# skitzoid/Box2D-MT

Hardware: AMD Instinct MI355X
Metric: world steps/sec at 99858 bodies per GPU (BASELINE config 3: Tumbler 100k, CCD off; Step = collide + island solve + broad-phase + state read-back); for N > 1: container-steps/s = world steps/s x N containers in the one sharded world (higher is better)
Workload: dtype f32

## Files before the change

### box2d-mt_amd/csrc/b2d_kernels_solve_large.h

```cpp
#ifndef B2D_KERNELS_SOLVE_LARGE_H
#define B2D_KERNELS_SOLVE_LARGE_H

#include "b2d_kernels_solve_small.h"

#define LC_WORDS ((int)(sizeof(ContactConstraint) / 4))
#define LC_VEL_WORDS 36
#define LC_IMP_FIRST 10
#define LC_MASS_FIRST 28
#define LC_POS_FIRST 36

__device__ __forceinline__ void lcStore(const DW& W, int row, const ContactConstraint& cc, int first, int last)
{
	uint32_t words[LC_WORDS];
	memcpy(words, &cc, sizeof(ContactConstraint));
	uint32_t* dst = (uint32_t*)W.lc;
#pragma unroll
	for (int f = 0; f < LC_WORDS; ++f)
	{
		if (f >= first && f < last) dst[(size_t)f * W.capContacts + row] = words[f];
	}
}

__device__ __forceinline__ void lcLoad(const DW& W, int row, ContactConstraint& cc, int first, int last)
{
// ... 345 lines not shown
	for (int s = blockIdx.x * blockDim.x + threadIdx.x; s < n; s += gridDim.x * blockDim.x)
	{
		if (W.li_color[s] >= 0) continue;
		const int ci = W.li_contacts[s];
		int4 ids = C.ids[ci];
		uint32_t pr = colorPriority(ci);
		if ((W.b_flags[ids.z] & BF_TYPE_MASK) != BT_STATIC) atomicMax(&W.bodyClaim[ids.z], pr);
		if ((W.b_flags[ids.w] & BF_TYPE_MASK) != BT_STATIC) atomicMax(&W.bodyClaim[ids.w], pr);
	}
}

__global__ __launch_bounds__(256) void k_color_resolve(DW W)
{
	b2dPhaseStamp(W);
	DState* S = W.st;
	if (S->c.nUncolored == 0) return;
	const int n = S->c.nLContacts;
	const ContactArrays& C = W.ca[S->cur];
	int colored = 0;
	for (int s = blockIdx.x * blockDim.x + threadIdx.x; s < n; s += gridDim.x * blockDim.x)
	{
		if (W.li_color[s] >= 0) continue;
		const int ci = W.li_contacts[s];
		int4 ids = C.ids[ci];
		uint32_t pr = colorPriority(ci);
		const bool nsA = (W.b_flags[ids.z] & BF_TYPE_MASK) != BT_STATIC;
		const bool nsB = (W.b_flags[ids.w] & BF_TYPE_MASK) != BT_STATIC;
		bool win = true;
		if (nsA && __hip_atomic_load(&W.bodyClaim[ids.z], __ATOMIC_RELAXED, __HIP_MEMORY_SCOPE_AGENT) != pr) win = false;
		if (nsB && __hip_atomic_load(&W.bodyClaim[ids.w], __ATOMIC_RELAXED, __HIP_MEMORY_SCOPE_AGENT) != pr) win = false;
		if (!win) continue;
		uint64_t used = colorClassMask(constraintIsCut(W, ids.z, nsA, ids.w, nsB)) | colorTestMask(W);
		if (nsA) used |= W.bodyColorMask[ids.z];
		if (nsB) used |= W.bodyColorMask[ids.w];
		int color = used == ~0ull ? MAX_COLORS - 1 : __ffsll((long long)~used) - 1;
		if (used == ~0ull) atomicOr(&S->c.overflow, 4);
		uint64_t bit = 1ull << color;
		if (nsA) { W.bodyColorMask[ids.z] |= bit; W.bodyClaim[ids.z] = 0; }
		if (nsB) { W.bodyColorMask[ids.w] |= bit; W.bodyClaim[ids.w] = 0; }
		W.li_color[s] = color;
		C.color[ci] = color;
		atomicAdd(&W.colorCount[colorSlot(color)], 1);
		atomicMax(&S->c.nColors, color + 1);
		noteColorUsed(S, color);
		++colored;
	}
	if (colored) atomicSub(&S->c.nUncolored, colored);
}

__host__ __device__ inline bool b2dColorAheadNoPartition(const Counters& c, int aheadMinRows)
{
	return aheadMinRows > 0 && c.nBlocks == 0 && c.nLContacts >= aheadMinRows;
}
__device__ __forceinline__ void colorSmallBody(const DW& W);
__global__ __launch_bounds__(1024) void k_color_small(DW W, int queuedAhead, int aheadMinRows, DState* pub, int pubSeq)
{
	b2dPhaseStamp(W);
	DState* S = W.st;
	if (threadIdx.x == 0) S->gapClock[2] = wall_clock64();
	bool run = true, publish = pub != nullptr;
	if (queuedAhead)
	{
		const bool noPart = b2dColorAheadNoPartition(S->c, aheadMinRows);
		run = b2dPartitionSettled(S->c) || noPart;
		publish = publish && noPart;
	}
	if (S->c.nUncolList > COLOR_SMALL_MAX || S->c.needRecolor) run = false;
	if (run) colorSmallBody(W);
	if (publish)
	{
		__syncthreads();
		if (run && threadIdx.x < MAX_COLORS) S->c.colorRows[threadIdx.x] = threadIdx.x == HUB_COLOR ? 0 : __hip_atomic_load(&W.colorCount[colorSlot(threadIdx.x)], __ATOMIC_RELAXED, __HIP_MEMORY_SCOPE_WORKGROUP);
		__syncthreads();
		b2dPublishCensus(W, pub, pubSeq);
	}
}
__device__ __forceinline__ void colorSmallBody(const DW& W)
{
	DState* S = W.st;
	const ContactArrays& C = W.ca[S->cur];
	__shared__ int s_left, s_colored, s_maxColor, s_n;
	if (threadIdx.x == 0)
	{
		s_n = S->c.nUncolList;
		s_maxColor = 0;
	}
	__syncthreads();
	{
		const int nc = S->c.nCompact + S->c.nUncolList <= COLOR_SMALL_MAX ? S->c.nCompact : 0;
		for (int k = threadIdx.x; k < nc; k += blockDim.x)
		{
			const int s = W.compactList[k];
			const int c = W.li_color[s];
			if (c <= 0 || c >= MAX_COLORS) continue;
			const int ci = W.li_contacts[s];
			const int4 ids = C.ids[ci];
			const bool nsA = (W.b_flags[ids.z] & BF_TYPE_MASK) != BT_STATIC;
			const bool nsB = (W.b_flags[ids.w] & BF_TYPE_MASK) != BT_STATIC;
			uint64_t used = colorClassMask(constraintIsCut(W, ids.z, nsA, ids.w, nsB)) | colorTestMask(W);
			if (nsA) used |= __hip_atomic_load((unsigned long long*)&W.bodyColorMask[ids.z], __ATOMIC_RELAXED, __HIP_MEMORY_SCOPE_WORKGROUP);
			if (nsB) used |= __hip_atomic_load((unsigned long long*)&W.bodyColorMask[ids.w], __ATOMIC_RELAXED, __HIP_MEMORY_SCOPE_WORKGROUP);
			if (used == ~0ull || __ffsll((long long)~used) - 1 >= c) continue;
			const int slot = atomicAdd(&s_n, 1);
			if (slot >= COLOR_SMALL_MAX) continue;
			const unsigned long long bit = 1ull << c;
			if (nsA) (void)__hip_atomic_fetch_and((unsigned long long*)&W.bodyColorMask[ids.z], ~bit, __ATOMIC_RELAXED, __HIP_MEMORY_SCOPE_WORKGROUP);
			if (nsB) (void)__hip_atomic_fetch_and((unsigned long long*)&W.bodyColorMask[ids.w], ~bit, __ATOMIC_RELAXED, __HIP_MEMORY_SCOPE_WORKGROUP);
			W.li_color[s] = -1;
			C.color[ci] = -1;
			(void)__hip_atomic_fetch_add(&W.colorCount[colorSlot(c)], -1, __ATOMIC_RELAXED, __HIP_MEMORY_SCOPE_WORKGROUP);
			W.uncolList[slot] = s;
		}
	}
	__syncthreads();
	const int n = s_n < COLOR_SMALL_MAX ? s_n : COLOR_SMALL_MAX;
	if (threadIdx.x == 0)
	{
		s_left = n;
		if (s_n > S->c.nUncolList) S->c.compactMoved = s_n - S->c.nUncolList;
	}
	constexpr int PER = COLOR_SMALL_MAX / 1024;
	int it_s[PER], it_ci[PER], it_a[PER], it_b[PER];
	uint32_t it_pr[PER];
	uint64_t it_class[PER];
	bool it_open[PER];
#pragma unroll
	for (int j = 0; j < PER; ++j)
	{
		const int k = (int)threadIdx.x + j * 1024;
		it_open[j] = false;
		it_s[j] = it_ci[j] = 0; it_a[j] = it_b[j] = -1; it_pr[j] = 0u; it_class[j] = 0ull;
		if (k < n)
		{
			const int s = W.uncolList[k];
			it_s[j] = s;
			it_open[j] = W.li_color[s] < 0;
			const int ci = W.li_contacts[s];
			it_ci[j] = ci;
			const int4 ids = C.ids[ci];
			const bool nsA = (W.b_flags[ids.z] & BF_TYPE_MASK) != BT_STATIC;
			const bool nsB = (W.b_flags[ids.w] & BF_TYPE_MASK) != BT_STATIC;
			it_a[j] = nsA ? ids.z : -1;
			it_b[j] = nsB ? ids.w : -1;
			it_pr[j] = colorPriority(ci);
			it_class[j] = colorClassMask(constraintIsCut(W, ids.z, nsA, ids.w, nsB)) | colorTestMask(W);
		}
	}
	__syncthreads();
	const int maxRounds = W.testColorRounds > 0 ? W.testColorRounds : 4 * MAX_COLORS;
	for (int round = 0; round < maxRounds && s_left > 0; ++round)
	{
		if (threadIdx.x == 0) s_colored = 0;
#pragma unroll
		for (int j = 0; j < PER; ++j)
		{
			if (!it_open[j]) continue;
			if (it_a[j] >= 0) (void)__hip_atomic_fetch_max(&W.bodyClaim[it_a[j]], it_pr[j], __ATOMIC_RELAXED, __HIP_MEMORY_SCOPE_WORKGROUP);
			if (it_b[j] >= 0) (void)__hip_atomic_fetch_max(&W.bodyClaim[it_b[j]], it_pr[j], __ATOMIC_RELAXED, __HIP_MEMORY_SCOPE_WORKGROUP);
		}
		__syncthreads();
		int colored = 0;
#pragma unroll
		for (int j = 0; j < PER; ++j)
		{
			if (!it_open[j]) continue;
			const int A = it_a[j], B = it_b[j];
			const uint32_t pr = it_pr[j];
			bool win = true;
			if (A >= 0 && __hip_atomic_load(&W.bodyClaim[A], __ATOMIC_RELAXED, __HIP_MEMORY_SCOPE_WORKGROUP) != pr) win = false;
			if (B >= 0 && __hip_atomic_load(&W.bodyClaim[B], __ATOMIC_RELAXED, __HIP_MEMORY_SCOPE_WORKGROUP) != pr) win = false;
			if (!win) continue;
			uint64_t used = it_class[j];
			if (A >= 0) used |= __hip_atomic_load((unsigned long long*)&W.bodyColorMask[A], __ATOMIC_RELAXED, __HIP_MEMORY_SCOPE_WORKGROUP);
			if (B >= 0) used |= __hip_atomic_load((unsigned long long*)&W.bodyColorMask[B], __ATOMIC_RELAXED, __HIP_MEMORY_SCOPE_WORKGROUP);
			const int color = used == ~0ull ? MAX_COLORS - 1 : __ffsll((long long)~used) - 1;
			if (used == ~0ull) atomicOr(&S->c.overflow, 4);
			const unsigned long long bit = 1ull << color;
			if (A >= 0) { (void)__hip_atomic_fetch_or((unsigned long long*)&W.bodyColorMask[A], bit, __ATOMIC_RELAXED, __HIP_MEMORY_SCOPE_WORKGROUP); __hip_atomic_store(&W.bodyClaim[A], 0u, __ATOMIC_RELAXED, __HIP_MEMORY_SCOPE_WORKGROUP); }
			if (B >= 0) { (void)__hip_atomic_fetch_or((unsigned long long*)&W.bodyColorMask[B], bit, __ATOMIC_RELAXED, __HIP_MEMORY_SCOPE_WORKGROUP); __hip_atomic_store(&W.bodyClaim[B], 0u, __ATOMIC_RELAXED, __HIP_MEMORY_SCOPE_WORKGROUP); }
			W.li_color[it_s[j]] = color;
			C.color[it_ci[j]] = color;
			(void)__hip_atomic_fetch_add(&W.colorCount[colorSlot(color)], 1, __ATOMIC_RELAXED, __HIP_MEMORY_SCOPE_WORKGROUP);
			atomicMax(&s_maxColor, color + 1);
			noteColorUsed(S, color);
			it_open[j] = false;
			++colored;
		}
		if (colored) atomicAdd(&s_colored, colored);
		__syncthreads();
		if (threadIdx.x == 0) s_left -= s_colored;
		__syncthreads();
	}
	if (threadIdx.x == 0)
	{
		int nc = S->c.nColors > s_maxColor ? S->c.nColors : s_maxColor;
		if (nc > MAX_COLORS) nc = MAX_COLORS;
		while (nc > 0 && __hip_atomic_load(&W.colorCount[colorSlot(nc - 1)], __ATOMIC_RELAXED, __HIP_MEMORY_SCOPE_WORKGROUP) == 0) --nc;
		S->c.nColors = nc;
		S->c.nUncolored = s_left;
		S->c.colorRounds += 1;
	}
}

__global__ void k_color_scan(DW W)
{
	b2dPhaseStamp(W);
	if (W.st->c.nColors <= MAX_COLORS)
	{
		if (blockIdx.x == 0 && threadIdx.x < 64)
		{
			const int c = (int)threadIdx.x;
			const int cnt = c < MAX_COLORS ? W.colorCount[colorSlot(c)] : 0;
			int incl = cnt;
			for (int off = 1; off < 64; off <<= 1)
			{
				const int o = __shfl_up(incl, off);
				if (c >= off) incl += o;
			}
			W.colorStart[c] = incl - cnt;
			if (c == 63) W.colorStart[64] = incl;
			if (c == HUB_COLOR) W.st->c.nHubRows = cnt;
		}
		return;
	}
	if (blockIdx.x == 0 && threadIdx.x == 0)
	{
		const int nc = W.st->c.nColors > MAX_COLORS ? W.st->c.nColors : MAX_COLORS;
		int run = 0;
		for (int c = 0; c <= nc; ++c)
		{
			W.colorStart[c] = run;
			if (c < nc) run += W.colorCount[colorSlot(c)];
		}
		W.st->c.nHubRows = W.colorCount[colorSlot(HUB_COLOR)];
	}
}

__global__ __launch_bounds__(256) void k_exact_begin(DW W)
{
	b2dPhaseStamp(W);
	DState* S = W.st;
	const int n = S->c.nSContacts;
	for (int c = blockIdx.x * blockDim.x + threadIdx.x; c <= n; c += gridDim.x * blockDim.x)
	{
		W.colorCount[colorSlot(c)] = 0;
		W.colorCursor[colorSlot(c)] = 0;
	}
	if (blockIdx.x == 0 && threadIdx.x == 0) S->c.nColors = 0;
}

__global__ __launch_bounds__(256) void k_exact_convert(DW W)
{
	b2dPhaseStamp(W);
	DState* S = W.st;
// ... 1182 lines not shown
```

### box2d-mt_amd/csrc/b2d_world.h

```cpp
#ifndef B2D_WORLD_H
#define B2D_WORLD_H

#include "b2d_solver.h"
#include "b2d_joint.h"
#include "b2d_wave.h"

#define BF_TYPE_MASK 0x3u
#define BF_AWAKE 0x4u
#define BF_AUTOSLEEP 0x8u
#define BF_BULLET 0x10u
#define BF_FIXEDROT 0x20u
#define BF_ACTIVE 0x40u
#define BF_ISLAND 0x80u
#define BF_LARGE 0x100u

#define BT_STATIC 0u
#define BT_KINEMATIC 1u
#define BT_DYNAMIC 2u

#define CF_TOUCHING 0x1u
#define CF_ENABLED 0x2u
#define CF_FILTER 0x4u
#define CF_TOI_CANDIDATE 0x8u
#define CF_SENSOR 0x10u
#define CF_DESTROY 0x20u
#define CF_ISLAND 0x40u
#define CF_TOI 0x80u
#define CF_TOI_LISTED 0x100u
#define CF_TOI_PENDING 0x200u
#define CF_REPORTED 0x400u
#define CF_PRESOLVE 0x800u
#define CF_VC_ONE_POINT 0x10000u
#define CF_USER_REJECT 0x20000u
#define CF_PRESOLVE_OFF 0x40000u
#define CF_FOREIGN 0x80000u
#define CF_TOI_COUNT_SHIFT 12
#define CF_TOI_COUNT_MASK 0xf000u
#define CF_TOI_STATE_MASK (CF_TOI | CF_TOI_LISTED | CF_TOI_PENDING | CF_TOI_COUNT_MASK)

#define PF_SENSOR 0x10000
#define PF_THICK 0x20000

#define SMALL_ISLAND_MAX_W 512
#define SMALL_CHUNK_LANES 1024
#define TINY_ISLAND_MAX_W 128
#define SMALL_ISLAND_MAX_JOINTS 64
#define TINY_CHUNK_LANES 256
#define MAX_COLORS 64
#define HUB_DEGREE 30
#define HUB_COLOR (MAX_COLORS - 1)
#define CENSUS_WG_MAX_BODIES 16384
#define COLOR_SMALL_MAX 4096
#define TOI_NEW_LIST_MAX 1024
#define COUNT_RANK_MAX 4096
#define SHARD_BIG_BODIES 4096
#define SHARD_BIG_MAX 1024
#define SHARD_MAX_RANKS 8
#define SHARD_BODY_WORDS 13
#define SHARD_CONTACT_WORDS 5
#define SHARD_JOINT_WORDS 6
#define CUT_COLOR_BASE 32
#define BLOCK_LANES 1024
#define ROOT_PEN_SLOTS 5
#define BLOCK_MAX_BODIES 1024
#define MAX_BLOCKS 1024
#define BLK_SLOT 32
#define BLOCK_TARGET_DEG 1500

struct ContactArrays
{
	int4* ids;
	uint64_t* key;
	uint32_t* flags;
	float4* mat;
	float4* man0;
	float4* man1;
	float4* imp;
	int4* man3;
	int* color;
	int* mgr;
};

#define KS_KEPT 0
#define KS_CAUSE_INVALID 1
#define KS_CAUSE_STALE 2
#define KS_CAUSE_MASK 3
#define KS_CAUSE_FILL 4
#define KS_CAUSE_SHARDED 5
#define KS_CAUSE_OFF 6
#define KS_TOMBSTONES 7
#define KS_INSERTS 8
#define KS_NOT_FOUND 9
#define KS_STATS 10

struct Counters
{
	int nContacts;
	int nDestroy;
	int nTouching;
	int nMoves;
	int nMovesSeen;
	int candRounds[32];
	int nPairs;
	int nNewContacts;
	int nRoots;
// ... 192 lines not shown
	GearRec* gears;
	int* jadjStart;
	int* jadj;
	int* rootJointStart;
	int* rootJointCursor;
	int* lj_list;
	int* rootJointOkay;

	int* parent;
	int* rootSeed;
	int* rootBodies;
	int* rootContacts;
	int* rootJoints;
	int4* rootScanIn;
	int4* rootScanOut;
	int* rootIsland;
	int* deg;
	int* adjStart;
	int* adjCursor;
	int* adj;
	int2* adjSlot;
	int* si_root;
	int* si_bodyStart;
	int* si_contactStart;
	int* si_wStart;
	int* si_maxLevel;
	int* si_bodies;
	int* si_contacts;
	int* si_level;
	int* si_stack;
	int* si_lastLevel;
	int* b_slot;
	int* b_island;
	int* chunkFirst;
	int* li_bodies;
	int* li_contacts;
	int* li_roots;
	int* li_color;
	int* colorCount;
	int* colorStart;
	int* colorCursor;
	int* compactList;
	int* uncolList;
	int* hubRowOf;
	float4* hubDelta;
	int* hubList;
	unsigned long long* hubMeta;
	unsigned long long* hubFirst;
	int hubWide;
	int* li_sorted;
	int4* li_ref;
	uint32_t* bodyClaim;
	uint64_t* bodyColorMask;
	uint64_t* bodyActive;
	float4* solveSnapBody;
	float4* solveSnapImp; uint32_t* solveSnapCFlags;
	struct JointRec* solveSnapJoints; struct GearRec* solveSnapGears;
	uint64_t* bodyRest;
	int eventsOn;
	unsigned long long* evKey;
	int4* evInfo;
	int* dfRank;
	float4* dfInbox;
	float4* b_posv;
	float* lc;
	int* b_rowDirty;
	float4* warmDelta;
	uint32_t* rootPen;
	int* rootDone;
	uint32_t* rootSleepMin;
	int* b_blk1;
	int* b_adopt;
	int* b_adoptStage;
	int* blkRows;
	int* blkRowStart;
	int* blkCursor;
	int* blkBodyCount;
	int* blkBodyCursor;
	int* blkBodyStart;
	int* blkBodies;
	int* rowColor;
	float4* b_cutv;
	int blockSort;
	int shardRank, shardCount;
	int* bigRoots;
	int spatial;
	uint8_t* b_owner;
	uint8_t* spNewOwner;
	uint8_t* spAwake;
	int spFullRows;
	int* spStraddle;
	int capStraddle;
	int* spCount;
	int* spTarget;
	int* spOwnOut;
	int spOwnCap;
	int4* spTailKey;
	int userFilter;
	int preSolveOn, postSolveOn;
	float4* pre_o0;
	float4* pre_o1;
	float4* pre_oimp;
	int4* pre_o3;
	PreSolveRec* preRecs;
	PostSolveRec* postRecs;
	ToiLogRec* toiLog;
// ... 200 lines not shown
```

### box2d-mt_amd/csrc/b2hip_api_callbacks.h

```cpp

int b2hip_set_contact_filter(b2hip_world* w, b2hip_should_collide_fn fn, void* user)
{
	if (int rcu = checkUsable(w, "b2hip_set_contact_filter", true)) return rcu;
	w->filterFn = fn;
	w->filterUser = user;
	w->dw.userFilter = hasFilter(w) ? 1 : 0;
	return B2HIP_OK;
}

int b2hip_set_contact_filter_batch(b2hip_world* w, b2hip_should_collide_batch_fn fn, void* user)
{
	if (int rcu = checkUsable(w, "b2hip_set_contact_filter_batch", true)) return rcu;
	w->filterBatchFn = fn;
	if (fn) w->filterUser = user;
	w->dw.userFilter = hasFilter(w) ? 1 : 0;
	return B2HIP_OK;
}

int b2hip_default_should_collide(b2hip_world* w, int fixture_a, int fixture_b)
{
	if (!w || fixture_a < 0 || fixture_b < 0 || fixture_a >= (int)w->fixtures.size() || fixture_b >= (int)w->fixtures.size())
		return setError(B2HIP_ERR_INVALID, "bad fixture id");
	const HostFixture& a = w->fixtures[fixture_a];
	const HostFixture& b = w->fixtures[fixture_b];
// ... 163 lines not shown
	case 4: src = w->b_flags.p; elem = 4; break;
	case 5: src = w->b_damp.p; break;
	case 6: src = w->b_mass.p; break;
	case 7: src = w->d_state.p; elem = 4; break;
	case 8: src = w->dbgPreVel.p; break;
	case 9: src = w->dbgVel.p; break;
	case 10: src = w->dbgLi.p; elem = 4; break;
	case 11: src = w->gridBar.p; elem = 4; break;
	case 12:
	{
		if (first < 0 || count < 0 || first + count > COLOR_SLOT_PADDED) return setError(B2HIP_ERR_INVALID, "colour census: [0, 65)");
		HIP_TRY(hipStreamSynchronize(w->stream));
		if (count > 0) HIP_TRY(hipMemcpy2D(out, sizeof(int), w->colorCount.p + colorSlot(first), COLOR_SLOT_STRIDE * sizeof(int), sizeof(int), (size_t)count, hipMemcpyDeviceToHost));
		return 0;
	}
	case 13: src = w->bodyColorMask.p; elem = 8; break;
	case 14: src = w->deg.p; elem = 4; break;
	case 15: src = w->hubList.p; elem = 4; break;
	case 16: src = w->bodyActive.p; elem = 8; break;
	case 17: src = w->b_blk1.p; elem = 4; break;
	case 18: src = w->li_ref.p; break;
	case 19: src = w->rowColor.p; elem = 4; break;
	case 20: src = w->blkRowStart.p; elem = 4; break;
	case 21: src = w->bodyRest.p; elem = 8; break;
	case 22:
	{
		const long long stats[2] = { w->statSorts, w->statSortsOnepass };
		if (first < 0 || count < 0 || first + count > 2) return setError(B2HIP_ERR_INVALID, "pair-update statistics: [0, 2)");
		memcpy(out, stats + first, (size_t)count * sizeof(long long));
		return 0;
	}
	case 23:
	{
		if (first < 0 || count < 0 || first + count > KS_STATS + 2) return setError(B2HIP_ERR_INVALID, "key-set statistics: [0, 12)");
		Counters c;
		HIP_TRY(hipMemcpy(&c, &w->d_state.p->c, sizeof(Counters), hipMemcpyDeviceToHost));
		long long stats[KS_STATS + 2];
		for (int k = 0; k < KS_STATS; ++k) stats[k] = (long long)c.ksStats[k];
		stats[KS_STATS] = c.ksFill;
		stats[KS_STATS + 1] = c.ksMask;
		memcpy(out, stats + first, (size_t)count * sizeof(long long));
		return 0;
	}
	case 24:
	{
		if (first != 0 || count != 1) return setError(B2HIP_ERR_INVALID, "narrow-phase statistics: [0, 1)");
		memcpy(out, &w->statCollideCompact, sizeof(long long));
		return 0;
	}
	case 31:
	{
		if (first != 0 || count != 1) return setError(B2HIP_ERR_INVALID, "island-build statistics: [0, 1)");
		memcpy(out, &w->statUnionSkipped, sizeof(long long));
		return 0;
	}
	case 29:
	{
		if (first != 0 || count != 1) return setError(B2HIP_ERR_INVALID, "lifecycle statistics: [0, 1)");
		memcpy(out, &w->statLifecycleLongSorts, sizeof(long long));
		return 0;
	}
	case 30:
	{
		const long long stats[2] = { w->statFixtureLongSorts, w->statFixtureRelists };
		if (first < 0 || count < 0 || first + count > 2) return setError(B2HIP_ERR_INVALID, "fixture-batch statistics: [0, 2)");
		memcpy(out, stats + first, (size_t)count * sizeof(long long));
		return 0;
	}
	case 25:
	{
		if (first < 0 || count < 0 || first + count > ToiStats::N) return setError(B2HIP_ERR_INVALID, "TOI host statistics: [0, 10)");
		memcpy(out, w->toiStats.n + first, (size_t)count * sizeof(long long));
		return 0;
	}
	case 26:
	{
		const int nb = (int)std::min(w->bodies.size(), w->upBodies);
		if (first < 0 || count < 0 || first + count > nb) return setError(B2HIP_ERR_INVALID, "effective blocks: [0, uploaded bodies)");
		if (count == 0) return 0;
		if (!w->d_state.p || !w->b_blk1.p || !w->b_adopt.p || !w->b_flags.p) return setError(B2HIP_ERR_INVALID, "effective blocks: nothing uploaded yet");
		Counters c;
		HIP_TRY(hipMemcpy(&c, &w->d_state.p->c, sizeof(Counters), hipMemcpyDeviceToHost));
		std::vector<int> blk1((size_t)count), adopt((size_t)count);
		std::vector<uint32_t> flags((size_t)count);
		HIP_TRY(hipMemcpy(blk1.data(), w->b_blk1.p + first, (size_t)count * sizeof(int), hipMemcpyDeviceToHost));
		HIP_TRY(hipMemcpy(adopt.data(), w->b_adopt.p + first, (size_t)count * sizeof(int), hipMemcpyDeviceToHost));
		HIP_TRY(hipMemcpy(flags.data(), w->b_flags.p + first, (size_t)count * sizeof(uint32_t), hipMemcpyDeviceToHost));
		const int blocks = c.nBlocks < MAX_BLOCKS ? c.nBlocks : MAX_BLOCKS;
		const bool ownIdOff = (w->dw.nJoints != 0 || c.maxDegree > HUB_DEGREE) && w->dw.noOwnIdBlocks >= 0;
		int* e = (int*)out;
		for (int k = 0; k < count; ++k)
		{
			const int offered = adopt[k] & 0x7ff;
			if (blk1[k]) e[k] = blk1[k];
			else if (offered || w->dw.noOwnIdBlocks > 0) e[k] = offered;
			else if ((flags[k] & BF_LARGE) == 0 || ownIdOff) e[k] = 0;
			else e[k] = blocks > 0 ? ownIdBlock(first + k, blocks) : 0;
		}
		return 0;
	}
	case 27:
	{
		const int N = 28;
		if (first < 0 || count < 0 || first + count > N) return setError(B2HIP_ERR_INVALID, "large-island plan: [0, 28)");
		const b2hip_world::PlanRecord& r = w->planRecord;
		Counters c;
// ... 292 lines not shown
```

### box2d-mt_amd/csrc/b2hip_host_world.h

```cpp

static thread_local std::string g_lastError;

static int setError(int code, const std::string& msg)
{
	g_lastError = msg;
	return code;
}

#define HIP_TRY(expr)                                                                                   \
	do                                                                                                  \
	{                                                                                                   \
		hipError_t _e = (expr);                                                                         \
		if (_e != hipSuccess)                                                                           \
		{                                                                                               \
			return setError(B2HIP_ERR_HIP, std::string(#expr) + ": " + hipGetErrorString(_e));          \
		}                                                                                               \
	} while (0)

static void (*g_rcclDestroy)(void* comm) = nullptr;

static std::atomic<long long> g_liveBlocks{0};

template <typename T>
struct DevArray
// ... 182 lines not shown
	X(int, p_key, z.np, true, true) \
	X(uint32_t, p_filter0, z.np, true, true) \
	X(int, p_filter1, z.np, true, true) \
	X(float2, p_mat, z.np, true, true) \
	X(int, b_proxyHead, z.nb, true, true) \
	X(int, p_next, z.np, true, true) \
	 \
	X(RevoluteJoint, solveSnapJoints, w->recoverOn ? z.nj : 1, true, true) \
	X(GearRec, solveSnapGears, w->recoverOn ? z.ng : 1, true, true) \
	X(int, jadjStart, z.nb + 2, true, true) \
	X(int, jadj, 2 * w->joints.size() + 2, true, true) \
	X(int, rootJointStart, z.nb + 2, true, true) \
	X(int, rootJointCursor, z.nb, true, true) \
	X(int, lj_list, w->joints.size() + 2, true, true) \
	X(int, rootJointOkay, z.nb, true, true) \
	X(int, parent, z.nb, true, true) \
	X(int, rootSeed, z.nb, true, true) \
	X(int, rootBodies, z.nb, true, true) \
	X(int, rootContacts, z.nb, true, true) \
	X(int, rootJoints, z.nb, true, true) \
	X(int, rootIsland, z.nb, true, true) \
	X(int, deg, z.nb + 1, true, true) \
	X(int, adjStart, z.nb + 2, true, true) \
	X(int, adjCursor, z.nb, true, true) \
	X(int, adj, 2 * z.cc, true, true) \
	X(int2, adjSlot, z.cc, true, true) \
	X(int4, rootScanIn, z.nb + 1, true, true) \
	X(int4, rootScanOut, z.nb + 2, true, true) \
	X(int, si_root, z.nb + 1, true, true) \
	X(int, si_bodyStart, z.nb + 2, true, true) \
	X(int, si_contactStart, z.nb + 2, true, true) \
	X(int, si_wStart, z.nb + 2, true, true) \
	X(int, si_maxLevel, z.nb + 1, true, true) \
	X(int, si_bodies, z.nb, true, true) \
	X(int, si_contacts, z.cc, true, true) \
	X(int, si_level, z.cc, true, true) \
	X(int, si_stack, z.nb, true, true) \
	X(int, si_lastLevel, z.nb, true, true) \
	X(int, b_slot, z.nb, true, true) \
	X(int, b_island, z.nb, true, true) \
	X(int, chunkFirst, (z.nb + z.cc) / (TINY_CHUNK_LANES / 2) + 4, true, true) \
	X(int, li_bodies, z.nb, true, true) \
	X(int, li_contacts, z.cc, true, true) \
	X(int, li_roots, z.nb, true, true) \
	X(int, li_color, z.cc, true, true) \
	 \
	X(int, colorCount, z.cc + 2 + COLOR_SLOT_PADDED * COLOR_SLOT_STRIDE, true, true) \
	X(int, colorStart, z.cc + 2, true, true) \
	X(int, colorCursor, z.cc + 2 + COLOR_SLOT_PADDED * COLOR_SLOT_STRIDE, true, true) \
	X(int, li_sorted, z.cc, true, true) \
	X(int4, li_ref, z.cc, true, true) \
	X(uint32_t, bodyClaim, z.nb, true, true) \
	X(uint64_t, bodyColorMask, z.nb, true, true) \
	X(uint64_t, bodyActive, z.nb, true, true) \
	X(uint64_t, bodyRest, z.nb, true, true) \
	X(float4, b_posv, z.nb, true, true) \
	X(unsigned long long, evKey, z.cc, true, true) \
	X(int4, evInfo, z.cc, true, true) \
	X(int, uncolList, COLOR_SMALL_MAX, true, true) \
	X(int, compactList, COLOR_SMALL_MAX, true, true) \
	X(int, hubRowOf, z.cc, true, true) \
	X(int, hubList, z.cc, true, true) \
	X(float4, hubDelta, z.cc, true, true) \
	X(unsigned long long, hubMeta, 8, true, true) \
	X(unsigned long long, hubFirst, z.nb, true, true) \
	X(float4, solveSnapBody, w->recoverOn ? 6 * z.nb : 1, true, true) \
	X(float4, solveSnapImp, w->recoverOn ? z.cc : 1, true, true) \
	X(uint32_t, solveSnapCFlags, w->recoverOn ? z.cc : 1, true, true) \
	X(uint32_t, rootPen, ROOT_PEN_SLOTS * z.nb, true, true) \
	X(int, rootDone, z.nb, true, true) \
	X(uint32_t, rootSleepMin, z.nb, true, true) \
	X(float, lc, (size_t)LC_WORDS * z.cc, false, false) \
	X(float4, warmDelta, 4 * z.cc, false, false)  \
	X(int, moveBuf, 2 * z.np + 64, true, true) \
	X(int, gridCount, z.gridSize, true, true) \
	X(int, gridStart, z.gridSize + 2, true, true) \
	X(int, gridCursor, z.gridSize, true, true) \
	X(int, gridItems, z.np, true, true) \
	X(float4, gridFat, z.np, true, true) \
	X(unsigned long long, arriveTree, (size_t)ARRIVE_SITES * TREE_WORDS, true, true) \
	X(int, largeProxies, z.np, true, true) \
	X(int, largeMoves, 2 * z.np + 64, true, true) \
	X(uint64_t, pairKey, z.capPairs, true, true) \
	X(uint64_t, pairKey2, z.capPairs, true, true) \
	X(int2, pairProxy, z.capPairs, true, true) \
	X(int2, pairProxy2, z.capPairs, true, true) \
	X(int, pairFirst, z.capPairs + 1, true, true) \
	X(int, pairRank, z.capPairs + 2, true, true) \
	X(int, radixHist, RADIX_DIGITS * z.radixTiles + 2, true, true) \
	X(int, scanTmp, 3 * (std::max(z.maxScanN, RADIX_DIGITS * z.radixTiles) / SCAN_TILE + 8), true, true) \
	X(int, keepFlag, z.cc + 1, true, true) \
	X(int, keepScan, z.cc + 2, true, true) \
	X(int, toiList, z.cc, true, true) \
	X(int, toiPos2c, z.cc, true, true) \
	X(int, toiDestroyList, z.cc, true, true) \
	X(int, toiNewList, TOI_NEW_LIST_MAX, true, true) \
	X(int, b_toiGroup, z.nb, true, true) \
	X(int, toiGroups, z.nb, true, true) \
	X(int, toiGroupCount, std::min<size_t>(z.nb, TOI_GROUPS_MAX), true, true) \
	X(int, toiGroupList, std::min<size_t>(z.nb, TOI_GROUPS_MAX) * CHAIN_ADJ_MAX, true, true) \
	X(int, toiMoved, TOI_MOVED_ALL_MAX, true, true) \
	X(int, toiNew, 8 * TOI_NEWPAIR_MAX, true, true) \
	X(int, toiParent, z.nb, true, true) \
	X(int, toiDomOf, z.nb, true, true) \
	X(int, toiDomRoot, TOI_DOMAINS_MAX, true, true) \
	X(int, toiDomCount, TOI_DOMAINS_MAX, true, true) \
// ... 729 lines not shown
{
	DW& d = w->dw;
	w->debugSync = envSet("B2HIP_DEBUG");
	w->traceLaunches = envSet("B2HIP_TRACE_LAUNCHES");
	w->debugTrace = envSet("B2HIP_TRACE");
	w->forceLarge = envInt("B2HIP_FORCE_LARGE", 0);
	w->kernelTimingLaunches = envSet("B2HIP_SOLVER_LAUNCHES");
	w->noSideStream = envSet("B2HIP_NO_SIDE_STREAM");
	w->profileDetail = envInt("B2HIP_PROFILE_DETAIL", 1) != 0;
	if (const char* e = getenv("B2HIP_SOLID_ROUNDS")) { const int v = atoi(e); w->solidRoundsEnv = (v == 1 || v == 2 || v == 4 || v == 8) ? v : 0; }
	w->collideSplitEnv = envInt("B2HIP_COLLIDE_SPLIT", -1);
	w->collideCompactOn = envInt("B2HIP_COLLIDE_COMPACT", 1) != 0;
	w->collideUnionOn = envInt("B2HIP_COLLIDE_UNION", 1) != 0;
	w->collideChunk = std::min(std::max(envInt("B2HIP_TEST_COLLIDE_CHUNK", 256), 1), 256);
	w->lifecycleSortMax = std::min(std::max(envInt("B2HIP_TEST_LIFECYCLE_SORT_MAX", LIFECYCLE_SORT_MAX), 0), LIFECYCLE_SORT_MAX);
	w->fixtureListRoom = std::max(envInt("B2HIP_TEST_FIXTURE_LIST_ROOM", -1), -1);
	w->collideUniOff = envInt("B2HIP_COLLIDE_UNI", 1) == 0;
	w->collideSortEnv = envInt("B2HIP_COLLIDE_SORT", -1);
	w->sortOnepass = envInt("B2HIP_SORT_ONEPASS", 1) != 0;
	d.keysetKeep = envInt("B2HIP_KEYSET_KEEP", 1) != 0 ? 1 : 0;
	d.keysetMaxFill = std::min(std::max(envInt("B2HIP_KEYSET_MAX_FILL", 37), 1), 90);
	w->collideStage = envInt("B2HIP_COLLIDE_STAGE", -1);
	w->noSweepBlocks = envSet("B2HIP_NO_SWEEP_BLOCKS");
	w->tracePartition = envSet("B2HIP_TRACE_PARTITION");
	w->traceRecovery = envSet("B2HIP_TRACE_RECOVERY");
	if (const char* e = getenv("B2HIP_GRID_HALF")) { w->gridForced = true; w->gridHalf = atoi(e) != 0; d.gridHalf = w->gridHalf ? 1 : 0; }
	d.noChainCreate = envSet("B2HIP_TOI_NO_CHAIN_CREATE") ? 1 : 0;
	d.noOwnIdBlocks = envSet("B2HIP_NO_OWN_ID_BLOCKS") ? 1 : envSet("B2HIP_OWN_ID_BLOCKS_ALL") ? -1 : 0;
	w->noBlocks = envSet("B2HIP_NO_BLOCKS");
	w->blockLanes = 0;
	if (const char* e = getenv("B2HIP_BLOCK_LANES")) w->blockLanes = atoi(e) == 512 ? 512 : (atoi(e) == 256 ? 256 : (atoi(e) == 1024 ? 1024 : 0));
	w->toiSw.serialOnly = envSet("B2HIP_TOI_SERIAL");
	w->toiSw.syncOnly = envSet("B2HIP_TOI_SYNC");
	w->toiSw.domWideOnly = envSet("B2HIP_TOI_DOM_WIDE");
	w->toiSw.noSpecDomains = envSet("B2HIP_TOI_NO_SPEC_DOMAINS");
	w->toiSw.assumeFreshGrid = envSet("B2HIP_DEBUG_ASSUME_FRESH_GRID");
	w->toiSw.noDomains = envSet("B2HIP_TOI_NO_DOMAINS");
	w->toiSw.why = envSet("B2HIP_TOI_WHY");
	w->handoverWhy = envSet("B2HIP_HANDOVER_WHY");
	w->shardTrace = envOn("B2HIP_SHARD_TRACE");
	w->recoverOn = !envOn("B2HIP_NO_RECOVER");
	w->noCensusPoll = envOn("B2HIP_NO_CENSUS_POLL");
	w->noStatePoll = envOn("B2HIP_NO_STATE_POLL");
	w->lazyReadback = envOn("B2HIP_LAZY_READBACK");
	w->earlyRowsMin = envInt("B2HIP_EARLY_ROWS_MIN", w->earlyRowsMin);
	w->stepDeadlineS = getenv("B2HIP_STEP_DEADLINE_S") ? atof(getenv("B2HIP_STEP_DEADLINE_S")) : 300.0;
	w->pollDelayUs = envInt("B2HIP_TEST_POLL_DELAY_US", 0);
	d.bigChunks = envSet("B2HIP_BIG_CHUNKS") ? 1 : 0;
	d.smallMaxW = TINY_ISLAND_MAX_W;
	if (const char* e = getenv("B2HIP_SMALL_MAX_W")) d.smallMaxW = std::max(1, std::min((int)SMALL_ISLAND_MAX_W, atoi(e)));
	d.noFreeBodies = envOn("B2HIP_NO_FREE_BODIES") ? 1 : 0;
	d.testMaxColors = envInt("B2HIP_TEST_MAX_COLORS", 0);
	d.testColorRounds = envInt("B2HIP_TEST_COLOR_ROUNDS", 0);
	d.testSpinMax = std::max(0, envInt("B2HIP_TEST_SPIN_MAX", 0));
	d.restPoll = getenv("B2HIP_REST_POLL") ? std::max(1, std::min(16, atoi(getenv("B2HIP_REST_POLL")))) : 1;
	d.hubSerial = envOn("B2HIP_HUB_SERIAL") ? 1 : 0;
	w->hubWaves = envInt("B2HIP_HUB_WAVES", 0) == 1 ? 1 : 8;
	w->sweepEnd = !envOn("B2HIP_NO_SWEEP_END") && !envSet("B2HIP_HUB_WAVES");
	w->sweepTail = w->sweepEnd && !envOn("B2HIP_NO_TAIL");
	w->sweepStamps = envSet("B2HIP_SWEEP_STAMPS");
	w->rowMarks = envOn("B2HIP_ROW_MARKS_CHECK") ? 2 : envOn("B2HIP_NO_ROW_MARKS") ? 0 : 1;
	w->bodyWarm = !envOn("B2HIP_NO_BODY_WARM");
	w->restFlow = w->sweepEnd && !envOn("B2HIP_NO_REST");
	w->noHubBuild = envOn("B2HIP_NO_HUB_BUILD");
	w->noHubOrder = envOn("B2HIP_NO_HUB_ORDER");
	w->hubOrderAll = envOn("B2HIP_HUB_ORDER");
	if (getenv("B2HIP_SWEEP_ROWS_MAX")) w->sweepRowsMax = std::max(1, atoi(getenv("B2HIP_SWEEP_ROWS_MAX")));
	w->restHub = getenv("B2HIP_REST_HUB") ? std::max(0, std::min(2, atoi(getenv("B2HIP_REST_HUB")))) : 2;
	w->restRowsMax = getenv("B2HIP_REST_ROWS") ? std::min(atoi(getenv("B2HIP_REST_ROWS")), REST_ROWS_MAX - COLOR_SMALL_MAX) : 65536;
	w->tailRowsMax = envInt("B2HIP_TAIL_ROWS", SWEEP_END_LANES);
	d.hubWide = (w->sweepEnd && !d.hubSerial && envInt("B2HIP_HUB_WIDE", 1) != 0) ? 1 : 0;
}

struct WorldSizes
{
	const b2hip_world* w;
	size_t needContacts;
	size_t nb = std::max<size_t>(w->bodies.size(), 1), np = std::max<size_t>(w->fixtures.size(), 1);
	size_t nj = std::max<size_t>(w->joints.size(), 1), ng = std::max<size_t>(w->gears.size(), 1);
	size_t capPairs = std::max<size_t>(std::max<size_t>(8 * np + 4096, w->pairKey.cap), w->pairCapHint);
	size_t capContacts = std::max<size_t>(needContacts + capPairs, 1024);
	size_t cc = w->c_ids[0].capFor(capContacts);
	size_t gridSize = (size_t)nextPow2(2 * np);
	size_t maxScanN = std::max(std::max(nb + 2, gridSize + 2), std::max(cc + 2, capPairs + 2));
	size_t radixTiles = capPairs / RADIX_TILE + 2;
	size_t onepassTiles = w->sortOnepass ? std::min<size_t>(radixTiles, RADIX_ONEPASS_MAX_TILES) : 0;
	size_t collideChunks = w->collideCompactOn ? cc / (size_t)w->collideChunk + 2 : 0;
	size_t nPre = hasPreSolve(w) ? cc : 1, nPost = w->postSolveOn ? cc : 1, nFil = hasFilter(w) ? cc : 1;
};

static int ensureCapacity(b2hip_world* w, size_t needContacts)
{
	hipStream_t s = w->stream;
	const WorldSizes z = { w, needContacts };
	const size_t nb = z.nb;
	DW& d = w->dw;
	int rc = 0;
#define ENS(arr, n) do { rc = w->arr.ensure((n), s); if (rc) return rc; } while (0)
	ENS(d_state, 1);
	ENS(d_shapes, std::max<size_t>(w->shapes.size(), 1));
	ENS(d_joints, z.nj);
	ENS(d_gears, z.ng);
	d.shapes = w->d_shapes.p; d.joints = w->d_joints.p; d.gears = w->d_gears.p;
	for (int k = 0; k < 2; ++k)
	{
		ENS(c_ids[k], z.capContacts); ENS(c_key[k], z.capContacts); ENS(c_flags[k], z.capContacts); ENS(c_mat[k], z.capContacts);
// ... 77 lines not shown
```

Measured before the change: 386.1.

## Run small-batch graph coloring in LDS with a per-block body hash table

Adds an LDS variant of k_color_small. The bodies touched by the uncolored and compacted contacts are mapped into a shared-memory open-addressed hash table, and the claim/mask rounds run on LDS atomics instead of global atomics on bodyClaim and bodyColorMask. Masks and per-colour counts are written back to global memory once at the end. It falls back to the old global path when the table overflows, and adds a stats buffer that thread 0 updates on every launch. The LDS footprint is large (about 128 KB of shared arrays), which may fail to fit or limit occupancy, though only one block runs.

New measurement: 387.0 (median of 4 runs). About the same (+0.2%).

```diff
diff --git a/box2d-mt_amd/csrc/b2d_kernels_solve_large.h b/box2d-mt_amd/csrc/b2d_kernels_solve_large.h
--- a/box2d-mt_amd/csrc/b2d_kernels_solve_large.h
+++ b/box2d-mt_amd/csrc/b2d_kernels_solve_large.h
@@ -421,7 +421,9 @@
 {
 	return aheadMinRows > 0 && c.nBlocks == 0 && c.nLContacts >= aheadMinRows;
 }
-__device__ __forceinline__ void colorSmallBody(const DW& W);
+struct ColorSmallNote { int rounds, bodies, items; };
+__device__ __forceinline__ void colorSmallBody(const DW& W, ColorSmallNote* note);
+__device__ __forceinline__ bool colorSmallLds(const DW& W, ColorSmallNote* note);
 __global__ __launch_bounds__(1024) void k_color_small(DW W, int queuedAhead, int aheadMinRows, DState* pub, int pubSeq)
 {
 	b2dPhaseStamp(W);
@@ -435,7 +437,22 @@
 		publish = publish && noPart;
 	}
 	if (S->c.nUncolList > COLOR_SMALL_MAX || S->c.needRecolor) run = false;
-	if (run) colorSmallBody(W);
+	if (run)
+	{
+		__shared__ ColorSmallNote s_note;
+		const bool inLds = W.colorSmallLds && colorSmallLds(W, &s_note);
+		if (!inLds) colorSmallBody(W, &s_note);
+		if (threadIdx.x == 0)
+		{
+			unsigned long long* st = W.colorLdsStats;
+			const unsigned long long r = (unsigned long long)s_note.rounds, b = (unsigned long long)s_note.bodies, it = (unsigned long long)s_note.items;
+			st[inLds ? 0 : W.colorSmallLds ? 2 : 1] += 1ull;
+			st[3] += r; if (r > st[4]) st[4] = r;
+			if (inLds) { st[5] += b; if (b > st[6]) st[6] = b; }
+			st[7] += it; if (it > st[8]) st[8] = it;
+			if (it) st[9] += 1ull;
+		}
+	}
 	if (publish)
 	{
 		__syncthreads();
@@ -444,7 +461,7 @@
 		b2dPublishCensus(W, pub, pubSeq);
 	}
 }
-__device__ __forceinline__ void colorSmallBody(const DW& W)
+__device__ __forceinline__ void colorSmallBody(const DW& W, ColorSmallNote* note)
 {
 	DState* S = W.st;
 	const ContactArrays& C = W.ca[S->cur];
@@ -517,8 +534,10 @@
 	}
 	__syncthreads();
 	const int maxRounds = W.testColorRounds > 0 ? W.testColorRounds : 4 * MAX_COLORS;
+	int rounds = 0;
 	for (int round = 0; round < maxRounds && s_left > 0; ++round)
 	{
+		++rounds;
 		if (threadIdx.x == 0) s_colored = 0;
 #pragma unroll
 		for (int j = 0; j < PER; ++j)
@@ -568,7 +587,199 @@
 		S->c.nColors = nc;
 		S->c.nUncolored = s_left;
 		S->c.colorRounds += 1;
-	}
+		note->rounds = rounds;
+		note->bodies = 0;
+		note->items = n;
+	}
+}
+
+__device__ __forceinline__ bool colorSmallLds(const DW& W, ColorSmallNote* note)
+{
+	static_assert((COLOR_LDS_SLOTS & (COLOR_LDS_SLOTS - 1)) == 0 && COLOR_LDS_MAX_BODIES + 1024 < COLOR_LDS_SLOTS, "every lane may have one insert in flight when the count passes the limit");
+	DState* S = W.st;
+	const ContactArrays& C = W.ca[S->cur];
+	__shared__ int s_key[COLOR_LDS_SLOTS];
+	__shared__ uint32_t s_claim[COLOR_LDS_SLOTS];
+	__shared__ unsigned long long s_mask[COLOR_LDS_SLOTS];
+	__shared__ int s_cc[MAX_COLORS];
+	__shared__ unsigned long long s_used;
+	__shared__ int s_left, s_n, s_bodies, s_fail;
+	for (int i = threadIdx.x; i < COLOR_LDS_SLOTS; i += blockDim.x) { s_key[i] = -1; s_claim[i] = 0u; }
+	if (threadIdx.x < MAX_COLORS) s_cc[threadIdx.x] = 0;
+	const int n0 = S->c.nUncolList;
+	if (threadIdx.x == 0) { s_n = n0; s_bodies = 0; s_fail = 0; s_used = 0ull; }
+	__syncthreads();
+	const int cap = W.colorLdsBodies;
+	auto slotOf = [&](int body) -> int
+	{
+		if (__hip_atomic_load(&s_bodies, __ATOMIC_RELAXED, __HIP_MEMORY_SCOPE_WORKGROUP) > cap) { s_fail = 1; return 0; }
+		const uint32_t h = ((uint32_t)body * 2654435761u) >> 16;
+		for (int probe = 0; probe < COLOR_LDS_SLOTS; ++probe)
+		{
+			const int slot = (int)((h + (uint32_t)probe) & (uint32_t)(COLOR_LDS_SLOTS - 1));
+			int cur = __hip_atomic_load(&s_key[slot], __ATOMIC_RELAXED, __HIP_MEMORY_SCOPE_WORKGROUP);
+			if (cur == -1)
+			{
+				cur = atomicCAS(&s_key[slot], -1, body);
+				if (cur == -1)
+				{
+					s_mask[slot] = W.bodyColorMask[body];
+					if (atomicAdd(&s_bodies, 1) + 1 > cap) s_fail = 1;
+					return slot;
+				}
+			}
+			if (cur == body) return slot;
+		}
+		s_fail = 1;
+		return 0;
+	};
+	constexpr int PER = COLOR_SMALL_MAX / 1024;
+	int it_s[PER], it_ci[PER], it_a[PER], it_b[PER];
+	uint32_t it_pr[PER];
+	uint64_t it_class[PER];
+	bool it_open[PER];
+#pragma unroll
+	for (int j = 0; j < PER; ++j)
+	{
+		it_open[j] = false;
+		it_s[j] = it_ci[j] = 0; it_a[j] = it_b[j] = -1; it_pr[j] = 0u; it_class[j] = 0ull;
+	}
+	auto head = [&](int lo, int hi)
+	{
+#pragma unroll
+		for (int j = 0; j < PER; ++j)
+		{
+			const int k = (int)threadIdx.x + j * 1024;
+			if (k < lo || k >= hi) continue;
+			const int s = W.uncolList[k];
+			it_s[j] = s;
+			it_open[j] = W.li_color[s] < 0;
+			const int ci = W.li_contacts[s];
+			it_ci[j] = ci;
+			const int4 ids = C.ids[ci];
+			const bool nsA = (W.b_flags[ids.z] & BF_TYPE_MASK) != BT_STATIC;
+			const bool nsB = (W.b_flags[ids.w] & BF_TYPE_MASK) != BT_STATIC;
+			it_a[j] = nsA ? slotOf(ids.z) : -1;
+			it_b[j] = nsB ? slotOf(ids.w) : -1;
+			it_pr[j] = colorPriority(ci);
+			it_class[j] = colorClassMask(constraintIsCut(W, ids.z, nsA, ids.w, nsB)) | colorTestMask(W);
+		}
+	};
+	head(0, n0);
+	const int nc = S->c.nCompact + n0 <= COLOR_SMALL_MAX ? S->c.nCompact : 0;
+	for (int k = threadIdx.x; k < nc; k += blockDim.x)
+	{
+		const int s = W.compactList[k];
+		const int c = W.li_color[s];
+		if (c <= 0 || c >= MAX_COLORS) continue;
+		const int4 ids = C.ids[W.li_contacts[s]];
+		if ((W.b_flags[ids.z] & BF_TYPE_MASK) != BT_STATIC) (void)slotOf(ids.z);
+		if ((W.b_flags[ids.w] & BF_TYPE_MASK) != BT_STATIC) (void)slotOf(ids.w);
+	}
+	__syncthreads();
+	if (s_fail) return false;
+	for (int k = threadIdx.x; k < nc; k += blockDim.x)
+	{
+		const int s = W.compactList[k];
+		const int c = W.li_color[s];
+		if (c <= 0 || c >= MAX_COLORS) continue;
+		const int ci = W.li_contacts[s];
+		const int4 ids = C.ids[ci];
+		const bool nsA = (W.b_flags[ids.z] & BF_TYPE_MASK) != BT_STATIC;
+		const bool nsB = (W.b_flags[ids.w] & BF_TYPE_MASK) != BT_STATIC;
+		const int sa = nsA ? slotOf(ids.z) : -1, sb = nsB ? slotOf(ids.w) : -1;
+		uint64_t used = colorClassMask(constraintIsCut(W, ids.z, nsA, ids.w, nsB)) | colorTestMask(W);
+		if (sa >= 0) used |= s_mask[sa];
+		if (sb >= 0) used |= s_mask[sb];
+		if (used == ~0ull || __ffsll((long long)~used) - 1 >= c) continue;
+		const int slot = atomicAdd(&s_n, 1);
+		if (slot >= COLOR_SMALL_MAX) continue;
+		const unsigned long long bit = 1ull << c;
+		if (sa >= 0) (void)atomicAnd(&s_mask[sa], ~bit);
+		if (sb >= 0) (void)atomicAnd(&s_mask[sb], ~bit);
+		W.li_color[s] = -1;
+		C.color[ci] = -1;
+		(void)atomicAdd(&s_cc[c], -1);
+		W.uncolList[slot] = s;
+	}
+	__syncthreads();
+	const int n = s_n < COLOR_SMALL_MAX ? s_n : COLOR_SMALL_MAX;
+	if (threadIdx.x == 0)
+	{
+		s_left = n;
+		if (s_n > n0) S->c.compactMoved = s_n - n0;
+	}
+	head(n0, n);
+	__syncthreads();
+	const int maxRounds = W.testColorRounds > 0 ? W.testColorRounds : 4 * MAX_COLORS;
+	int rounds = 0;
+	uint64_t myColors = 0ull;
+	for (int round = 0; round < maxRounds && s_left > 0; ++round)
+	{
+		++rounds;
+#pragma unroll
+		for (int j = 0; j < PER; ++j)
+		{
+			if (!it_open[j]) continue;
+			if (it_a[j] >= 0) (void)atomicMax(&s_claim[it_a[j]], it_pr[j]);
+			if (it_b[j] >= 0) (void)atomicMax(&s_claim[it_b[j]], it_pr[j]);
+		}
+		__syncthreads();
+		int colored = 0;
+#pragma unroll
+		for (int j = 0; j < PER; ++j)
+		{
+			if (!it_open[j]) continue;
+			const int A = it_a[j], B = it_b[j];
+			const uint32_t pr = it_pr[j];
+			bool win = true;
+			if (A >= 0 && __hip_atomic_load(&s_claim[A], __ATOMIC_RELAXED, __HIP_MEMORY_SCOPE_WORKGROUP) != pr) win = false;
+			if (B >= 0 && __hip_atomic_load(&s_claim[B], __ATOMIC_RELAXED, __HIP_MEMORY_SCOPE_WORKGROUP) != pr) win = false;
+			if (!win) continue;
+			uint64_t used = it_class[j];
+			if (A >= 0) used |= s_mask[A];
+			if (B >= 0) used |= s_mask[B];
+			const int color = used == ~0ull ? MAX_COLORS - 1 : __ffsll((long long)~used) - 1;
+			if (used == ~0ull) atomicOr(&S->c.overflow, 4);
+			const unsigned long long bit = 1ull << color;
+			if (A >= 0) { s_mask[A] |= bit; __hip_atomic_store(&s_claim[A], 0u, __ATOMIC_RELAXED, __HIP_MEMORY_SCOPE_WORKGROUP); }
+			if (B >= 0) { s_mask[B] |= bit; __hip_atomic_store(&s_claim[B], 0u, __ATOMIC_RELAXED, __HIP_MEMORY_SCOPE_WORKGROUP); }
+			W.li_color[it_s[j]] = color;
+			C.color[it_ci[j]] = color;
+			(void)atomicAdd(&s_cc[color], 1);
+			myColors |= bit;
+			it_open[j] = false;
+			++colored;
+		}
+		if (colored) (void)atomicSub(&s_left, colored);
+		__syncthreads();
+	}
+	if (myColors) (void)atomicOr(&s_used, myColors);
+	__syncthreads();
+	for (int i = threadIdx.x; i < COLOR_LDS_SLOTS; i += blockDim.x)
+	{
+		const int body = s_key[i];
+		if (body >= 0) W.bodyColorMask[body] = s_mask[i];
+	}
+	if (threadIdx.x < MAX_COLORS && s_cc[threadIdx.x] != 0) (void)__hip_atomic_fetch_add(&W.colorCount[colorSlot(threadIdx.x)], s_cc[threadIdx.x], __ATOMIC_RELAXED, __HIP_MEMORY_SCOPE_WORKGROUP);
+	__syncthreads();
+	if (threadIdx.x == 0)
+	{
+		const unsigned long long used = s_used;
+		if ((uint32_t)used) atomicOr(&S->c.colorMaskLo, (uint32_t)used);
+		if ((uint32_t)(used >> 32)) atomicOr(&S->c.colorMaskHi, (uint32_t)(used >> 32));
+		const int maxColor = used ? 64 - __clzll((long long)used) : 0;
+		int ncol = S->c.nColors > maxColor ? S->c.nColors : maxColor;
+		if (ncol > MAX_COLORS) ncol = MAX_COLORS;
+		while (ncol > 0 && __hip_atomic_load(&W.colorCount[colorSlot(ncol - 1)], __ATOMIC_RELAXED, __HIP_MEMORY_SCOPE_WORKGROUP) == 0) --ncol;
+		S->c.nColors = ncol;
+		S->c.nUncolored = s_left;
+		S->c.colorRounds += 1;
+		note->rounds = rounds;
+		note->bodies = s_bodies;
+		note->items = n;
+	}
+	return true;
 }
 
 __global__ void k_color_scan(DW W)
diff --git a/box2d-mt_amd/csrc/b2d_world.h b/box2d-mt_amd/csrc/b2d_world.h
--- a/box2d-mt_amd/csrc/b2d_world.h
+++ b/box2d-mt_amd/csrc/b2d_world.h
@@ -51,6 +51,9 @@
 #define HUB_COLOR (MAX_COLORS - 1)
 #define CENSUS_WG_MAX_BODIES 16384
 #define COLOR_SMALL_MAX 4096
+#define COLOR_LDS_SLOTS 8192
+#define COLOR_LDS_MAX_BODIES 6144
+#define COLOR_LDS_STATS 10
 #define TOI_NEW_LIST_MAX 1024
 #define COUNT_RANK_MAX 4096
 #define SHARD_BIG_BODIES 4096
@@ -349,6 +352,9 @@
 	int4* li_ref;
 	uint32_t* bodyClaim;
 	uint64_t* bodyColorMask;
+	int colorSmallLds;
+	int colorLdsBodies;
+	unsigned long long* colorLdsStats;
 	uint64_t* bodyActive;
 	float4* solveSnapBody;
 	float4* solveSnapImp; uint32_t* solveSnapCFlags;
diff --git a/box2d-mt_amd/csrc/b2hip_api_callbacks.h b/box2d-mt_amd/csrc/b2hip_api_callbacks.h
--- a/box2d-mt_amd/csrc/b2hip_api_callbacks.h
+++ b/box2d-mt_amd/csrc/b2hip_api_callbacks.h
@@ -239,6 +239,14 @@
 	{
 		if (first != 0 || count != 1) return setError(B2HIP_ERR_INVALID, "island-build statistics: [0, 1)");
 		memcpy(out, &w->statUnionSkipped, sizeof(long long));
+		return 0;
+	}
+	case 32:
+	{
+		if (first < 0 || count < 0 || first + count > COLOR_LDS_STATS) return setError(B2HIP_ERR_INVALID, "k_color_small statistics: [0, 10)");
+		long long stats[COLOR_LDS_STATS] = {};
+		if (w->colorLdsStats.p) HIP_TRY(hipMemcpy(stats, w->colorLdsStats.p, sizeof(stats), hipMemcpyDeviceToHost));
+		memcpy(out, stats + first, (size_t)count * sizeof(long long));
 		return 0;
 	}
 	case 29:
diff --git a/box2d-mt_amd/csrc/b2hip_host_world.h b/box2d-mt_amd/csrc/b2hip_host_world.h
--- a/box2d-mt_amd/csrc/b2hip_host_world.h
+++ b/box2d-mt_amd/csrc/b2hip_host_world.h
@@ -258,6 +258,7 @@
 	X(int4, li_ref, z.cc, true, true) \
 	X(uint32_t, bodyClaim, z.nb, true, true) \
 	X(uint64_t, bodyColorMask, z.nb, true, true) \
+	X(unsigned long long, colorLdsStats, COLOR_LDS_STATS, true, true) \
 	X(uint64_t, bodyActive, z.nb, true, true) \
 	X(uint64_t, bodyRest, z.nb, true, true) \
 	X(float4, b_posv, z.nb, true, true) \
@@ -1093,6 +1094,8 @@
 	d.noFreeBodies = envOn("B2HIP_NO_FREE_BODIES") ? 1 : 0;
 	d.testMaxColors = envInt("B2HIP_TEST_MAX_COLORS", 0);
 	d.testColorRounds = envInt("B2HIP_TEST_COLOR_ROUNDS", 0);
+	d.colorSmallLds = envInt("B2HIP_COLOR_SMALL_LDS", 1) != 0 ? 1 : 0;
+	d.colorLdsBodies = std::max(1, std::min((int)COLOR_LDS_MAX_BODIES, envInt("B2HIP_TEST_COLOR_LDS_BODIES", COLOR_LDS_MAX_BODIES)));
 	d.testSpinMax = std::max(0, envInt("B2HIP_TEST_SPIN_MAX", 0));
 	d.restPoll = getenv("B2HIP_REST_POLL") ? std::max(1, std::min(16, atoi(getenv("B2HIP_REST_POLL")))) : 1;
 	d.hubSerial = envOn("B2HIP_HUB_SERIAL") ? 1 : 0;
```
